# ch4r10t33r/zigz

Hardware: AMD Instinct MI355X
Metric: trace steps/sec proved (BabyBear, 2^20 RV64I trace) (higher is better)
Workload: dtype u32

## Files before the change

### zigz_amd/csrc/host_sponge_batch.cpp

```cpp
#include <immintrin.h>
#include <stdint.h>
#include <stdlib.h>
#include <string.h>

#include <algorithm>
#include <atomic>
#include <condition_variable>
#include <deque>
#include <mutex>
#include <thread>
#include <vector>

#include "field.hpp"
#include "host_hash.hpp"

namespace zk {

bool cpu_has_avx512f();

namespace {

constexpr int SLOTS = 8;
constexpr size_t RATE = 136;

const uint64_t RC8[24] = {
    0x0000000000000001ull, 0x0000000000008082ull, 0x800000000000808aull, 0x8000000080008000ull, 0x000000000000808bull,
    0x0000000080000001ull, 0x8000000080008081ull, 0x8000000000008009ull, 0x000000000000008aull, 0x0000000000000088ull,
    0x0000000080008009ull, 0x000000008000000aull, 0x000000008000808bull, 0x800000000000008bull, 0x8000000000008089ull,
    0x8000000000008003ull, 0x8000000000008002ull, 0x8000000000000080ull, 0x000000000000800aull, 0x800000008000000aull,
    0x8000000080008081ull, 0x8000000000008080ull, 0x0000000080000001ull, 0x8000000080008008ull};

__attribute__((target("avx512f"))) void keccak_f1600_x8(uint64_t st[25][SLOTS]) {
#define X8_X3(a, b, c) _mm512_ternarylogic_epi64((a), (b), (c), 0x96)
#define X8_CHI(a, b, c) _mm512_ternarylogic_epi64((a), (b), (c), 0xD2)
#define X8_ROL(a, n) _mm512_rol_epi64((a), (n))
#define X8_B(n, a, cm, rp) X8_ROL(X8_X3(a, cm, rp), n)
#define X8_LD(i) _mm512_load_si512(st[i])
    __m512i a0 = X8_LD(0), a1 = X8_LD(1), a2 = X8_LD(2), a3 = X8_LD(3), a4 = X8_LD(4), a5 = X8_LD(5), a6 = X8_LD(6), a7 = X8_LD(7);
    __m512i a8 = X8_LD(8), a9 = X8_LD(9), a10 = X8_LD(10), a11 = X8_LD(11), a12 = X8_LD(12), a13 = X8_LD(13), a14 = X8_LD(14);
    __m512i a15 = X8_LD(15), a16 = X8_LD(16), a17 = X8_LD(17), a18 = X8_LD(18), a19 = X8_LD(19), a20 = X8_LD(20), a21 = X8_LD(21);
    __m512i a22 = X8_LD(22), a23 = X8_LD(23), a24 = X8_LD(24);
#pragma unroll 2
    for (int r = 0; r < 24; r++) {
        const __m512i c0 = X8_X3(X8_X3(a0, a5, a10), a15, a20), c1 = X8_X3(X8_X3(a1, a6, a11), a16, a21);
        const __m512i c2 = X8_X3(X8_X3(a2, a7, a12), a17, a22), c3 = X8_X3(X8_X3(a3, a8, a13), a18, a23);
        const __m512i c4 = X8_X3(X8_X3(a4, a9, a14), a19, a24);
        const __m512i r0 = X8_ROL(c0, 1), r1 = X8_ROL(c1, 1), r2 = X8_ROL(c2, 1), r3 = X8_ROL(c3, 1), r4 = X8_ROL(c4, 1);
        const __m512i b00 = X8_X3(a0, c4, r1);
        const __m512i b10 = X8_B(1, a1, c0, r2), b20 = X8_B(62, a2, c1, r3), b05 = X8_B(28, a3, c2, r4), b15 = X8_B(27, a4, c3, r0);
        const __m512i b16 = X8_B(36, a5, c4, r1), b01 = X8_B(44, a6, c0, r2), b11 = X8_B(6, a7, c1, r3), b21 = X8_B(55, a8, c2, r4);
        const __m512i b06 = X8_B(20, a9, c3, r0), b07 = X8_B(3, a10, c4, r1), b17 = X8_B(10, a11, c0, r2), b02 = X8_B(43, a12, c1, r3);
        const __m512i b12 = X8_B(25, a13, c2, r4), b22 = X8_B(39, a14, c3, r0), b23 = X8_B(41, a15, c4, r1), b08 = X8_B(45, a16, c0, r2);
        const __m512i b18 = X8_B(15, a17, c1, r3), b03 = X8_B(21, a18, c2, r4), b13 = X8_B(8, a19, c3, r0), b14 = X8_B(18, a20, c4, r1);
        const __m512i b24 = X8_B(2, a21, c0, r2), b09 = X8_B(61, a22, c1, r3), b19 = X8_B(56, a23, c2, r4), b04 = X8_B(14, a24, c3, r0);
        a0 = _mm512_xor_si512(X8_CHI(b00, b01, b02), _mm512_set1_epi64((long long)RC8[r]));
        a1 = X8_CHI(b01, b02, b03); a2 = X8_CHI(b02, b03, b04); a3 = X8_CHI(b03, b04, b00); a4 = X8_CHI(b04, b00, b01);
        a5 = X8_CHI(b05, b06, b07); a6 = X8_CHI(b06, b07, b08); a7 = X8_CHI(b07, b08, b09); a8 = X8_CHI(b08, b09, b05);
        a9 = X8_CHI(b09, b05, b06); a10 = X8_CHI(b10, b11, b12); a11 = X8_CHI(b11, b12, b13); a12 = X8_CHI(b12, b13, b14);
        a13 = X8_CHI(b13, b14, b10); a14 = X8_CHI(b14, b10, b11); a15 = X8_CHI(b15, b16, b17); a16 = X8_CHI(b16, b17, b18);
        a17 = X8_CHI(b17, b18, b19); a18 = X8_CHI(b18, b19, b15); a19 = X8_CHI(b19, b15, b16); a20 = X8_CHI(b20, b21, b22);
        a21 = X8_CHI(b21, b22, b23); a22 = X8_CHI(b22, b23, b24); a23 = X8_CHI(b23, b24, b20); a24 = X8_CHI(b24, b20, b21);
    }
#define X8_ST(i, v) _mm512_store_si512(st[i], (v))
    X8_ST(0, a0); X8_ST(1, a1); X8_ST(2, a2); X8_ST(3, a3); X8_ST(4, a4); X8_ST(5, a5); X8_ST(6, a6); X8_ST(7, a7); X8_ST(8, a8);
    X8_ST(9, a9); X8_ST(10, a10); X8_ST(11, a11); X8_ST(12, a12); X8_ST(13, a13); X8_ST(14, a14); X8_ST(15, a15); X8_ST(16, a16);
    X8_ST(17, a17); X8_ST(18, a18); X8_ST(19, a19); X8_ST(20, a20); X8_ST(21, a21); X8_ST(22, a22); X8_ST(23, a23); X8_ST(24, a24);
}

struct Job {
    uint64_t *st;
    size_t *pos;
    const uint8_t *tag;
    size_t tag_len;
    uint64_t start, count;
    std::mutex m;
    std::condition_variable cv;
    bool done = false;
};

struct Stream {
    static constexpr size_t CHUNK_RECORDS = 272;
    Job *job = nullptr;
    uint64_t v = 0, left = 0;
    size_t rec = 0, rd = 0, wr = 0;
    uint8_t tmpl[32];
    std::vector<uint8_t> buf;

    void open(Job *j) {
        job = j;
        rec = j->tag_len + 8;
        v = j->start % (uint64_t)P;
        left = j->count;
        rd = wr = 0;
        memset(tmpl, 0, sizeof(tmpl));
        memcpy(tmpl, j->tag, j->tag_len < 24 ? j->tag_len : 24);
        buf.resize(CHUNK_RECORDS * rec + RATE + 64);
    }
    size_t avail() const { return wr - rd; }
    bool exhausted() const { return left == 0 && rd == wr; }
    void fill() {
        if (avail() >= RATE || left == 0) return;
        if (rd) {
            memmove(buf.data(), buf.data() + rd, wr - rd);
            wr -= rd;
            rd = 0;
        }
        size_t m = (buf.size() - wr - 32) / rec;
        if (m > left) m = (size_t)left;
        uint8_t *q = buf.data() + wr;
        const size_t tl = job->tag_len;
        if (tl <= 24) {
            for (size_t k = 0; k < m; k++, q += rec) {
                memcpy(q, tmpl, 32);
                memcpy(q + tl, &v, 8);
                if (++v == (uint64_t)P) v = 0;
            }
        } else {
            for (size_t k = 0; k < m; k++, q += rec) {
                memcpy(q, job->tag, tl);
                memcpy(q + tl, &v, 8);
                if (++v == (uint64_t)P) v = 0;
            }
        }
        wr += m * rec;
        left -= m;
    }
};

class Service {
  public:
    ~Service() { resize(0); }

    void resize(int n) {
        std::unique_lock<std::mutex> lk(m_);
        if (n < 0) n = 0;
        if (n > 0 && !cpu_has_avx512f()) n = 0;
        if ((int)threads_.size() == n) return;
        enabled_.store(false, std::memory_order_release);
        stop_ = true;
        cv_.notify_all();
        std::vector<std::thread> old;
        old.swap(threads_);
        lk.unlock();
        for (auto &t : old) t.join();
        lk.lock();
        stop_ = false;
        for (int i = 0; i < n; i++) threads_.emplace_back([this] { serve(); });
        enabled_.store(n > 0, std::memory_order_release);
    }
    bool enabled() const { return enabled_.load(std::memory_order_acquire); }

    bool run(Job &j) {
        {
            std::lock_guard<std::mutex> lk(m_);
            if (threads_.empty() || stop_) return false;
            queue_.push_back(&j);
            pending_.fetch_add(1, std::memory_order_release);
        }
        cv_.notify_one();
        std::unique_lock<std::mutex> lk(j.m);
        j.cv.wait(lk, [&] { return j.done; });
        return true;
    }

  private:
    void serve() {
        alignas(64) uint64_t S[25][SLOTS];
        memset(S, 0, sizeof(S));
        Stream slot[SLOTS];
        size_t pos[SLOTS] = {0};
        int active = 0;
        for (;;) {
            if (active == 0 || (active < SLOTS && pending_.load(std::memory_order_acquire) > 0)) {
                std::unique_lock<std::mutex> lk(m_);
                if (active == 0) cv_.wait(lk, [&] { return stop_ || !queue_.empty(); });
                if (stop_ && active == 0 && queue_.empty()) return;
                for (int s = 0; s < SLOTS && !queue_.empty(); s++) {
                    if (slot[s].job) continue;
                    Job *j = queue_.front();
                    queue_.pop_front();
                    pending_.fetch_sub(1, std::memory_order_relaxed);
                    slot[s].open(j);
                    pos[s] = *j->pos;
                    for (int w = 0; w < 25; w++) S[w][s] = j->st[w];
                    active++;
                }
            }
            if (active == 1 && pending_.load(std::memory_order_acquire) == 0) {
                int s = 0;
                while (!slot[s].job) s++;
                Stream &st = slot[s];
                if (pos[s] == 0) {
                    uint64_t one[25];
                    for (int w = 0; w < 25; w++) one[w] = S[w][s];
                    for (int k = 0; k < 64; k++) {
                        st.fill();
                        if (st.avail() < RATE) break;
                        const uint8_t *src = st.buf.data() + st.rd;
                        for (int w = 0; w < 17; w++) {
                            uint64_t x;
                            memcpy(&x, src + 8 * w, 8);
                            one[w] ^= x;
                        }
                        st.rd += RATE;
                        host_keccak_permute(one, 0);
                    }
                    for (int w = 0; w < 25; w++) S[w][s] = one[w];
                }
            }
            bool permute = false;
            for (int s = 0; s < SLOTS; s++) {
                Stream &st = slot[s];
                if (!st.job) continue;
                st.fill();
                const size_t need = RATE - pos[s];
                size_t n = st.avail() < need ? st.avail() : need;
                const uint8_t *src = st.buf.data() + st.rd;
                if (pos[s] == 0 && n == RATE) {
                    for (int w = 0; w < 17; w++) {
                        uint64_t x;
                        memcpy(&x, src + 8 * w, 8);
                        S[w][s] ^= x;
                    }
                } else if (n) {
                    uint8_t blk[RATE] = {0};
                    memcpy(blk + pos[s], src, n);
                    for (int w = 0; w < 17; w++) {
                        uint64_t x;
                        memcpy(&x, blk + 8 * w, 8);
                        S[w][s] ^= x;
                    }
                }
                st.rd += n;
                pos[s] += n;
                if (pos[s] == RATE) {
                    pos[s] = 0;
                    permute = true;
                } else {
                    retire(S, s, slot, pos);
                    active--;
                }
            }
            if (permute) keccak_f1600_x8(S);
            for (int s = 0; s < SLOTS; s++)
                if (slot[s].job && slot[s].exhausted() && pos[s] == 0) {
                    retire(S, s, slot, pos);
                    active--;
                }
        }
    }

    static void retire(uint64_t S[25][SLOTS], int s, Stream *slot, size_t *pos) {
        Job *j = slot[s].job;
        for (int w = 0; w < 25; w++) j->st[w] = S[w][s];
        *j->pos = pos[s];
        slot[s].job = nullptr;
        std::lock_guard<std::mutex> lk(j->m);
        j->done = true;
        j->cv.notify_one();
    }

    std::mutex m_;
    std::condition_variable cv_;
    std::deque<Job *> queue_;
    std::vector<std::thread> threads_;
    bool stop_ = false;
    std::atomic<int> pending_{0};
    std::atomic<bool> enabled_{false};
};

Service &service() {
    static Service s;
    return s;
}

}

void host_sponge_servers(int n) { service().resize(n); }
bool host_sponge_batching() { return service().enabled(); }

bool host_sponge_absorb_tagged(uint64_t st[25], size_t *pos, const uint8_t *tag, size_t tag_len, uint64_t start, uint64_t count) {
    Job j;
    j.st = st;
    j.pos = pos;
    j.tag = tag;
    j.tag_len = tag_len;
    j.start = start;
    j.count = count;
    return service().run(j);
}

void host_keccak_permute_x8(uint64_t st[25][8]) { keccak_f1600_x8(st); }

void flat_commit_batch(const uint32_t *const *ev, const size_t *n, size_t count, uint8_t (*out)[32]) {
    constexpr size_t WORDS = RATE / 8;
    auto one = [&](size_t i) {
        Sha3_256 h;
        for (size_t j = 0; j < n[i]; j++) h.update_le64(ev[i][j]);
        h.finalize(out[i]);
    };
    std::vector<std::thread> th;
    if (!cpu_has_avx512f()) {
        th.reserve(count);
        for (size_t i = 0; i < count; i++) th.emplace_back(one, i);
        for (auto &t : th) t.join();
        return;
    }
    std::vector<size_t> order(count);
    for (size_t i = 0; i < count; i++) order[i] = i;
    std::sort(order.begin(), order.end(), [&](size_t a, size_t b) { return n[a] > n[b]; });
    auto group = [&](size_t g0) {
        const size_t ns = count - g0 < (size_t)SLOTS ? count - g0 : (size_t)SLOTS;
        alignas(64) uint64_t st[25][SLOTS];
        memset(st, 0, sizeof(st));
        size_t full[SLOTS] = {0};
        size_t blocks = 0;
        for (size_t s = 0; s < ns; s++) {
            full[s] = n[order[g0 + s]] / WORDS;
            if (full[s] > blocks) blocks = full[s];
        }
        auto finish = [&](size_t s) {
            const size_t i = order[g0 + s];
            Sha3_256 h;
            for (int l = 0; l < 25; l++) h.raw_state()[l] = st[l][s];
            *h.raw_pos() = 0;
            for (size_t j = full[s] * WORDS; j < n[i]; j++) h.update_le64(ev[i][j]);
            h.finalize(out[i]);
        };
        for (size_t s = 0; s < ns; s++)
            if (full[s] == 0) finish(s);
        for (size_t b = 0; b < blocks; b++) {
            for (size_t s = 0; s < ns; s++) {
                if (b >= full[s]) continue;
                const uint32_t *v = ev[order[g0 + s]] + b * WORDS;
                for (size_t w = 0; w < WORDS; w++) st[w][s] ^= v[w];
            }
            keccak_f1600_x8(st);
            for (size_t s = 0; s < ns; s++)
                if (full[s] == b + 1) finish(s);
        }
    };
    const size_t groups = (count + SLOTS - 1) / SLOTS;
    th.reserve(groups);
    for (size_t g = 1; g < groups; g++) th.emplace_back(group, g * SLOTS);
    group(0);
    for (auto &t : th) t.join();
}

}
```

Measured before the change: 2.182 billion.

## Generate tagged sponge input in AVX-512 registers instead of staging byte buffers

The batched host Keccak sponge server no longer materialises tagged counter records into per-stream byte buffers. Streams with short tags now produce each 64-bit input lane directly in registers, using a gather from a per-slot tag table plus shifts of the running counter. Several absorb-and-permute blocks then run back-to-back with the state held in registers, up to a cap set by an environment variable. This removes the memmove/memcpy staging and the per-block state reloads, at the cost of more complex lane arithmetic and a gather per lane.

```diff
diff --git a/zigz_amd/csrc/host_sponge_batch.cpp b/zigz_amd/csrc/host_sponge_batch.cpp
--- a/zigz_amd/csrc/host_sponge_batch.cpp
+++ b/zigz_amd/csrc/host_sponge_batch.cpp
@@ -30,41 +30,97 @@
     0x8000000000008003ull, 0x8000000000008002ull, 0x8000000000000080ull, 0x000000000000800aull, 0x800000008000000aull,
     0x8000000080008081ull, 0x8000000000008080ull, 0x0000000080000001ull, 0x8000000080008008ull};
 
-__attribute__((target("avx512f"))) void keccak_f1600_x8(uint64_t st[25][SLOTS]) {
 #define X8_X3(a, b, c) _mm512_ternarylogic_epi64((a), (b), (c), 0x96)
 #define X8_CHI(a, b, c) _mm512_ternarylogic_epi64((a), (b), (c), 0xD2)
 #define X8_ROL(a, n) _mm512_rol_epi64((a), (n))
 #define X8_B(n, a, cm, rp) X8_ROL(X8_X3(a, cm, rp), n)
-#define X8_LD(i) _mm512_load_si512(st[i])
-    __m512i a0 = X8_LD(0), a1 = X8_LD(1), a2 = X8_LD(2), a3 = X8_LD(3), a4 = X8_LD(4), a5 = X8_LD(5), a6 = X8_LD(6), a7 = X8_LD(7);
-    __m512i a8 = X8_LD(8), a9 = X8_LD(9), a10 = X8_LD(10), a11 = X8_LD(11), a12 = X8_LD(12), a13 = X8_LD(13), a14 = X8_LD(14);
-    __m512i a15 = X8_LD(15), a16 = X8_LD(16), a17 = X8_LD(17), a18 = X8_LD(18), a19 = X8_LD(19), a20 = X8_LD(20), a21 = X8_LD(21);
-    __m512i a22 = X8_LD(22), a23 = X8_LD(23), a24 = X8_LD(24);
+#define X8_LOAD(st)                                                                                                          \
+    __m512i a0 = _mm512_load_si512(st[0]), a1 = _mm512_load_si512(st[1]), a2 = _mm512_load_si512(st[2]);                      \
+    __m512i a3 = _mm512_load_si512(st[3]), a4 = _mm512_load_si512(st[4]), a5 = _mm512_load_si512(st[5]);                      \
+    __m512i a6 = _mm512_load_si512(st[6]), a7 = _mm512_load_si512(st[7]), a8 = _mm512_load_si512(st[8]);                      \
+    __m512i a9 = _mm512_load_si512(st[9]), a10 = _mm512_load_si512(st[10]), a11 = _mm512_load_si512(st[11]);                  \
+    __m512i a12 = _mm512_load_si512(st[12]), a13 = _mm512_load_si512(st[13]), a14 = _mm512_load_si512(st[14]);                \
+    __m512i a15 = _mm512_load_si512(st[15]), a16 = _mm512_load_si512(st[16]), a17 = _mm512_load_si512(st[17]);                \
+    __m512i a18 = _mm512_load_si512(st[18]), a19 = _mm512_load_si512(st[19]), a20 = _mm512_load_si512(st[20]);                \
+    __m512i a21 = _mm512_load_si512(st[21]), a22 = _mm512_load_si512(st[22]), a23 = _mm512_load_si512(st[23]);                \
+    __m512i a24 = _mm512_load_si512(st[24])
+#define X8_ST(st, i, v) _mm512_store_si512(st[i], (v))
+#define X8_STORE(st)                                                                                                         \
+    X8_ST(st, 0, a0); X8_ST(st, 1, a1); X8_ST(st, 2, a2); X8_ST(st, 3, a3); X8_ST(st, 4, a4); X8_ST(st, 5, a5);               \
+    X8_ST(st, 6, a6); X8_ST(st, 7, a7); X8_ST(st, 8, a8); X8_ST(st, 9, a9); X8_ST(st, 10, a10); X8_ST(st, 11, a11);           \
+    X8_ST(st, 12, a12); X8_ST(st, 13, a13); X8_ST(st, 14, a14); X8_ST(st, 15, a15); X8_ST(st, 16, a16); X8_ST(st, 17, a17);   \
+    X8_ST(st, 18, a18); X8_ST(st, 19, a19); X8_ST(st, 20, a20); X8_ST(st, 21, a21); X8_ST(st, 22, a22); X8_ST(st, 23, a23);   \
+    X8_ST(st, 24, a24)
+#define X8_ROUND(rc)                                                                                                         \
+    {                                                                                                                        \
+        const __m512i c0 = X8_X3(X8_X3(a0, a5, a10), a15, a20), c1 = X8_X3(X8_X3(a1, a6, a11), a16, a21);                     \
+        const __m512i c2 = X8_X3(X8_X3(a2, a7, a12), a17, a22), c3 = X8_X3(X8_X3(a3, a8, a13), a18, a23);                     \
+        const __m512i c4 = X8_X3(X8_X3(a4, a9, a14), a19, a24);                                                              \
+        const __m512i r0 = X8_ROL(c0, 1), r1 = X8_ROL(c1, 1), r2 = X8_ROL(c2, 1), r3 = X8_ROL(c3, 1), r4 = X8_ROL(c4, 1);     \
+        const __m512i b00 = X8_X3(a0, c4, r1);                                                                               \
+        const __m512i b10 = X8_B(1, a1, c0, r2), b20 = X8_B(62, a2, c1, r3), b05 = X8_B(28, a3, c2, r4);                      \
+        const __m512i b15 = X8_B(27, a4, c3, r0), b16 = X8_B(36, a5, c4, r1), b01 = X8_B(44, a6, c0, r2);                     \
+        const __m512i b11 = X8_B(6, a7, c1, r3), b21 = X8_B(55, a8, c2, r4), b06 = X8_B(20, a9, c3, r0);                      \
+        const __m512i b07 = X8_B(3, a10, c4, r1), b17 = X8_B(10, a11, c0, r2), b02 = X8_B(43, a12, c1, r3);                   \
+        const __m512i b12 = X8_B(25, a13, c2, r4), b22 = X8_B(39, a14, c3, r0), b23 = X8_B(41, a15, c4, r1);                  \
+        const __m512i b08 = X8_B(45, a16, c0, r2), b18 = X8_B(15, a17, c1, r3), b03 = X8_B(21, a18, c2, r4);                  \
+        const __m512i b13 = X8_B(8, a19, c3, r0), b14 = X8_B(18, a20, c4, r1), b24 = X8_B(2, a21, c0, r2);                    \
+        const __m512i b09 = X8_B(61, a22, c1, r3), b19 = X8_B(56, a23, c2, r4), b04 = X8_B(14, a24, c3, r0);                  \
+        a0 = _mm512_xor_si512(X8_CHI(b00, b01, b02), _mm512_set1_epi64((long long)(rc)));                                    \
+        a1 = X8_CHI(b01, b02, b03); a2 = X8_CHI(b02, b03, b04); a3 = X8_CHI(b03, b04, b00); a4 = X8_CHI(b04, b00, b01);       \
+        a5 = X8_CHI(b05, b06, b07); a6 = X8_CHI(b06, b07, b08); a7 = X8_CHI(b07, b08, b09); a8 = X8_CHI(b08, b09, b05);       \
+        a9 = X8_CHI(b09, b05, b06); a10 = X8_CHI(b10, b11, b12); a11 = X8_CHI(b11, b12, b13); a12 = X8_CHI(b12, b13, b14);    \
+        a13 = X8_CHI(b13, b14, b10); a14 = X8_CHI(b14, b10, b11); a15 = X8_CHI(b15, b16, b17); a16 = X8_CHI(b16, b17, b18);   \
+        a17 = X8_CHI(b17, b18, b19); a18 = X8_CHI(b18, b19, b15); a19 = X8_CHI(b19, b15, b16); a20 = X8_CHI(b20, b21, b22);   \
+        a21 = X8_CHI(b21, b22, b23); a22 = X8_CHI(b22, b23, b24); a23 = X8_CHI(b23, b24, b20); a24 = X8_CHI(b24, b20, b21);   \
+    }
+
+__attribute__((target("avx512f"))) void keccak_f1600_x8(uint64_t st[25][SLOTS]) {
+    X8_LOAD(st);
 #pragma unroll 2
-    for (int r = 0; r < 24; r++) {
-        const __m512i c0 = X8_X3(X8_X3(a0, a5, a10), a15, a20), c1 = X8_X3(X8_X3(a1, a6, a11), a16, a21);
-        const __m512i c2 = X8_X3(X8_X3(a2, a7, a12), a17, a22), c3 = X8_X3(X8_X3(a3, a8, a13), a18, a23);
-        const __m512i c4 = X8_X3(X8_X3(a4, a9, a14), a19, a24);
-        const __m512i r0 = X8_ROL(c0, 1), r1 = X8_ROL(c1, 1), r2 = X8_ROL(c2, 1), r3 = X8_ROL(c3, 1), r4 = X8_ROL(c4, 1);
-        const __m512i b00 = X8_X3(a0, c4, r1);
-        const __m512i b10 = X8_B(1, a1, c0, r2), b20 = X8_B(62, a2, c1, r3), b05 = X8_B(28, a3, c2, r4), b15 = X8_B(27, a4, c3, r0);
-        const __m512i b16 = X8_B(36, a5, c4, r1), b01 = X8_B(44, a6, c0, r2), b11 = X8_B(6, a7, c1, r3), b21 = X8_B(55, a8, c2, r4);
-        const __m512i b06 = X8_B(20, a9, c3, r0), b07 = X8_B(3, a10, c4, r1), b17 = X8_B(10, a11, c0, r2), b02 = X8_B(43, a12, c1, r3);
-        const __m512i b12 = X8_B(25, a13, c2, r4), b22 = X8_B(39, a14, c3, r0), b23 = X8_B(41, a15, c4, r1), b08 = X8_B(45, a16, c0, r2);
-        const __m512i b18 = X8_B(15, a17, c1, r3), b03 = X8_B(21, a18, c2, r4), b13 = X8_B(8, a19, c3, r0), b14 = X8_B(18, a20, c4, r1);
-        const __m512i b24 = X8_B(2, a21, c0, r2), b09 = X8_B(61, a22, c1, r3), b19 = X8_B(56, a23, c2, r4), b04 = X8_B(14, a24, c3, r0);
-        a0 = _mm512_xor_si512(X8_CHI(b00, b01, b02), _mm512_set1_epi64((long long)RC8[r]));
-        a1 = X8_CHI(b01, b02, b03); a2 = X8_CHI(b02, b03, b04); a3 = X8_CHI(b03, b04, b00); a4 = X8_CHI(b04, b00, b01);
-        a5 = X8_CHI(b05, b06, b07); a6 = X8_CHI(b06, b07, b08); a7 = X8_CHI(b07, b08, b09); a8 = X8_CHI(b08, b09, b05);
-        a9 = X8_CHI(b09, b05, b06); a10 = X8_CHI(b10, b11, b12); a11 = X8_CHI(b11, b12, b13); a12 = X8_CHI(b12, b13, b14);
-        a13 = X8_CHI(b13, b14, b10); a14 = X8_CHI(b14, b10, b11); a15 = X8_CHI(b15, b16, b17); a16 = X8_CHI(b16, b17, b18);
-        a17 = X8_CHI(b17, b18, b19); a18 = X8_CHI(b18, b19, b15); a19 = X8_CHI(b19, b15, b16); a20 = X8_CHI(b20, b21, b22);
-        a21 = X8_CHI(b21, b22, b23); a22 = X8_CHI(b22, b23, b24); a23 = X8_CHI(b23, b24, b20); a24 = X8_CHI(b24, b20, b21);
-    }
-#define X8_ST(i, v) _mm512_store_si512(st[i], (v))
-    X8_ST(0, a0); X8_ST(1, a1); X8_ST(2, a2); X8_ST(3, a3); X8_ST(4, a4); X8_ST(5, a5); X8_ST(6, a6); X8_ST(7, a7); X8_ST(8, a8);
-    X8_ST(9, a9); X8_ST(10, a10); X8_ST(11, a11); X8_ST(12, a12); X8_ST(13, a13); X8_ST(14, a14); X8_ST(15, a15); X8_ST(16, a16);
-    X8_ST(17, a17); X8_ST(18, a18); X8_ST(19, a19); X8_ST(20, a20); X8_ST(21, a21); X8_ST(22, a22); X8_ST(23, a23); X8_ST(24, a24);
+    for (int r = 0; r < 24; r++) X8_ROUND(RC8[r]);
+    X8_STORE(st);
+}
+
+constexpr size_t LANE_TAG = 24;
+constexpr size_t TAB = LANE_TAG + 8;
+struct Lanes {
+    alignas(64) uint64_t v[SLOTS];
+    alignas(64) uint64_t r8[SLOTS];
+    alignas(64) uint64_t tl8[SLOTS], rec8[SLOTS];
+    alignas(64) uint64_t tab[SLOTS][TAB];
+};
+
+__attribute__((target("avx512f"))) void absorb_run(uint64_t S[25][SLOTS], Lanes &L, __mmask8 ready, size_t blocks) {
+    const __m512i tl8 = _mm512_load_si512(L.tl8), rec8 = _mm512_load_si512(L.rec8);
+    const __m512i base = _mm512_setr_epi64(0, 8 * TAB, 16 * TAB, 24 * TAB, 32 * TAB, 40 * TAB, 48 * TAB, 56 * TAB);
+    const __m512i p = _mm512_set1_epi64((long long)P), one = _mm512_set1_epi64(1), step = _mm512_set1_epi64(64);
+    __m512i v = _mm512_load_si512(L.v), r8 = _mm512_load_si512(L.r8);
+    X8_LOAD(S);
+#define X8_ABSORB(a)                                                                                                         \
+    {                                                                                                                        \
+        const __m512i t = _mm512_mask_i64gather_epi64(_mm512_setzero_si512(), ready, _mm512_add_epi64(base, r8), L.tab, 1);  \
+        const __m512i up = _mm512_sub_epi64(tl8, r8);                                                                        \
+        __m512i v1 = _mm512_add_epi64(v, one);                                                                               \
+        v1 = _mm512_maskz_mov_epi64(_mm512_cmpneq_epi64_mask(v1, p), v1);                                                    \
+        const __m512i c = _mm512_ternarylogic_epi64(_mm512_sllv_epi64(v, up), _mm512_srlv_epi64(v, _mm512_sub_epi64(r8, tl8)), \
+                                                    _mm512_sllv_epi64(v1, _mm512_add_epi64(up, rec8)), 0xFE);                \
+        a = _mm512_mask_ternarylogic_epi64(a, ready, t, c, 0x1E);                                           \
+        r8 = _mm512_add_epi64(r8, step);                                                                                     \
+        const __mmask8 next = _mm512_cmpge_epu64_mask(r8, rec8);                                                             \
+        r8 = _mm512_mask_sub_epi64(r8, next, r8, rec8);                                                                      \
+        v = _mm512_mask_mov_epi64(v, next, v1);                                                                              \
+    }
+    for (size_t b = 0; b < blocks; b++) {
+        X8_ABSORB(a0) X8_ABSORB(a1) X8_ABSORB(a2) X8_ABSORB(a3) X8_ABSORB(a4) X8_ABSORB(a5) X8_ABSORB(a6) X8_ABSORB(a7)
+        X8_ABSORB(a8) X8_ABSORB(a9) X8_ABSORB(a10) X8_ABSORB(a11) X8_ABSORB(a12) X8_ABSORB(a13) X8_ABSORB(a14)
+        X8_ABSORB(a15) X8_ABSORB(a16)
+#pragma unroll 2
+        for (int r = 0; r < 24; r++) X8_ROUND(RC8[r]);
+    }
+    X8_STORE(S);
+    _mm512_mask_store_epi64(L.v, ready, v);
+    _mm512_mask_store_epi64(L.r8, ready, r8);
 }
 
 struct Job {
@@ -78,52 +134,67 @@
     bool done = false;
 };
 
+constexpr size_t MAX_TAG = 248;
+
 struct Stream {
-    static constexpr size_t CHUNK_RECORDS = 272;
     Job *job = nullptr;
-    uint64_t v = 0, left = 0;
-    size_t rec = 0, rd = 0, wr = 0;
+    uint64_t *v = nullptr, *r8 = nullptr;
+    uint64_t rem = 0;
+    size_t rec = 0;
+    bool lanes = false;
     uint8_t tmpl[32];
-    std::vector<uint8_t> buf;
-
-    void open(Job *j) {
+
+    void open(Job *j, Lanes &L, int s) {
         job = j;
-        rec = j->tag_len + 8;
-        v = j->start % (uint64_t)P;
-        left = j->count;
-        rd = wr = 0;
+        const size_t tl = j->tag_len;
+        rec = tl + 8;
+        v = &L.v[s];
+        r8 = &L.r8[s];
+        *v = j->start % (uint64_t)P;
+        *r8 = 0;
+        rem = j->count * rec;
+        lanes = tl <= LANE_TAG;
         memset(tmpl, 0, sizeof(tmpl));
-        memcpy(tmpl, j->tag, j->tag_len < 24 ? j->tag_len : 24);
-        buf.resize(CHUNK_RECORDS * rec + RATE + 64);
-    }
-    size_t avail() const { return wr - rd; }
-    bool exhausted() const { return left == 0 && rd == wr; }
-    void fill() {
-        if (avail() >= RATE || left == 0) return;
-        if (rd) {
-            memmove(buf.data(), buf.data() + rd, wr - rd);
-            wr -= rd;
-            rd = 0;
-        }
-        size_t m = (buf.size() - wr - 32) / rec;
-        if (m > left) m = (size_t)left;
-        uint8_t *q = buf.data() + wr;
+        memcpy(tmpl, j->tag, lanes ? tl : LANE_TAG);
+        L.tl8[s] = 8 * tl;
+        L.rec8[s] = 8 * rec;
+        if (lanes) {
+            uint8_t img[2 * TAB + 8] = {0};
+            memcpy(img, j->tag, tl);
+            memcpy(img + rec, j->tag, tl);
+            for (size_t r = 0; r < rec; r++) memcpy(&L.tab[s][r], img + r, 8);
+        }
+    }
+    void take(uint8_t *dst, size_t n) {
         const size_t tl = job->tag_len;
-        if (tl <= 24) {
-            for (size_t k = 0; k < m; k++, q += rec) {
-                memcpy(q, tmpl, 32);
-                memcpy(q + tl, &v, 8);
-                if (++v == (uint64_t)P) v = 0;
-            }
-        } else {
-            for (size_t k = 0; k < m; k++, q += rec) {
-                memcpy(q, job->tag, tl);
-                memcpy(q + tl, &v, 8);
-                if (++v == (uint64_t)P) v = 0;
-            }
-        }
-        wr += m * rec;
-        left -= m;
+        size_t r = (size_t)(*r8 >> 3);
+        uint64_t c = *v;
+        rem -= n;
+        while (n) {
+            size_t m = rec;
+            if (r == 0 && lanes && n >= sizeof(tmpl)) {
+                memcpy(dst, tmpl, sizeof(tmpl));
+                memcpy(dst + tl, &c, 8);
+            } else if (r == 0 && n >= rec) {
+                memcpy(dst, job->tag, tl);
+                memcpy(dst + tl, &c, 8);
+            } else {
+                uint8_t one[MAX_TAG + 8];
+                memcpy(one, job->tag, tl);
+                memcpy(one + tl, &c, 8);
+                m = rec - r < n ? rec - r : n;
+                memcpy(dst, one + r, m);
+            }
+            dst += m;
+            n -= m;
+            r += m;
+            if (r == rec) {
+                r = 0;
+                if (++c == (uint64_t)P) c = 0;
+            }
+        }
+        *v = c;
+        *r8 = 8 * r;
     }
 };
 
@@ -167,9 +238,15 @@
     void serve() {
         alignas(64) uint64_t S[25][SLOTS];
         memset(S, 0, sizeof(S));
+        Lanes L;
+        memset(&L, 0, sizeof(L));
+        for (int s = 0; s < SLOTS; s++) L.rec8[s] = 64;
         Stream slot[SLOTS];
         size_t pos[SLOTS] = {0};
         int active = 0;
+        size_t run_cap = 32;
+        if (const char *e = getenv("ZIGZ_SPONGE_RUN_CAP"))
+            if (atoi(e) > 0) run_cap = (size_t)atoi(e);
         for (;;) {
             if (active == 0 || (active < SLOTS && pending_.load(std::memory_order_acquire) > 0)) {
                 std::unique_lock<std::mutex> lk(m_);
@@ -180,7 +257,7 @@
                     Job *j = queue_.front();
                     queue_.pop_front();
                     pending_.fetch_sub(1, std::memory_order_relaxed);
-                    slot[s].open(j);
+                    slot[s].open(j, L, s);
                     pos[s] = *j->pos;
                     for (int w = 0; w < 25; w++) S[w][s] = j->st[w];
                     active++;
@@ -190,48 +267,47 @@
                 int s = 0;
                 while (!slot[s].job) s++;
                 Stream &st = slot[s];
-                if (pos[s] == 0) {
+                if (pos[s] == 0 && st.rem >= RATE) {
                     uint64_t one[25];
                     for (int w = 0; w < 25; w++) one[w] = S[w][s];
-                    for (int k = 0; k < 64; k++) {
-                        st.fill();
-                        if (st.avail() < RATE) break;
-                        const uint8_t *src = st.buf.data() + st.rd;
+                    uint8_t chunk[64 * RATE];
+                    const size_t nb = st.rem / RATE < 64 ? (size_t)(st.rem / RATE) : 64;
+                    st.take(chunk, nb * RATE);
+                    for (size_t k = 0; k < nb; k++) {
+                        const uint8_t *src = chunk + k * RATE;
                         for (int w = 0; w < 17; w++) {
                             uint64_t x;
                             memcpy(&x, src + 8 * w, 8);
                             one[w] ^= x;
                         }
-                        st.rd += RATE;
                         host_keccak_permute(one, 0);
                     }
                     for (int w = 0; w < 25; w++) S[w][s] = one[w];
-                }
-            }
+                    if (st.rem >= RATE) continue;
+                }
+            }
+            __mmask8 ready = 0;
+            size_t blocks = run_cap;
             bool permute = false;
             for (int s = 0; s < SLOTS; s++) {
                 Stream &st = slot[s];
                 if (!st.job) continue;
-                st.fill();
+                if (st.lanes && pos[s] == 0 && st.rem >= RATE) {
+                    ready |= (__mmask8)(1u << s);
+                    if (st.rem / RATE < blocks) blocks = (size_t)(st.rem / RATE);
+                    continue;
+                }
                 const size_t need = RATE - pos[s];
-                size_t n = st.avail() < need ? st.avail() : need;
-                const uint8_t *src = st.buf.data() + st.rd;
-                if (pos[s] == 0 && n == RATE) {
-                    for (int w = 0; w < 17; w++) {
-                        uint64_t x;
-                        memcpy(&x, src + 8 * w, 8);
-                        S[w][s] ^= x;
-                    }
-                } else if (n) {
+                const size_t n = st.rem < need ? (size_t)st.rem : need;
+                if (n) {
                     uint8_t blk[RATE] = {0};
-                    memcpy(blk + pos[s], src, n);
+                    st.take(blk + pos[s], n);
                     for (int w = 0; w < 17; w++) {
                         uint64_t x;
                         memcpy(&x, blk + 8 * w, 8);
                         S[w][s] ^= x;
                     }
                 }
-                st.rd += n;
                 pos[s] += n;
                 if (pos[s] == RATE) {
                     pos[s] = 0;
@@ -241,9 +317,16 @@
                     active--;
                 }
             }
-            if (permute) keccak_f1600_x8(S);
+            if (ready) {
+                if (permute) blocks = 1;
+                absorb_run(S, L, ready, blocks);
+                for (int s = 0; s < SLOTS; s++)
+                    if (ready >> s & 1) slot[s].rem -= blocks * RATE;
+            } else if (permute) {
+                keccak_f1600_x8(S);
+            }
             for (int s = 0; s < SLOTS; s++)
-                if (slot[s].job && slot[s].exhausted() && pos[s] == 0) {
+                if (slot[s].job && slot[s].rem == 0 && pos[s] == 0) {
                     retire(S, s, slot, pos);
                     active--;
                 }
@@ -280,6 +363,7 @@
 bool host_sponge_batching() { return service().enabled(); }
 
 bool host_sponge_absorb_tagged(uint64_t st[25], size_t *pos, const uint8_t *tag, size_t tag_len, uint64_t start, uint64_t count) {
+    if (tag_len > MAX_TAG) return false;
     Job j;
     j.st = st;
     j.pos = pos;
```

Result: faster. 2.309 billion, median of 6 (+5.8%).

## Generate sponge blocks directly from precomputed shapes and batch multi-block Keccak runs

Applied to the files above, without the earlier changes.

Drops the buffered record stream and its memmove/memcpy refill. Each rate block is now synthesized directly with AVX-512 shifts from per-offset precomputed templates (BlockShape). A new run_blocks loop keeps all 8 sponge states in registers across up to 32 absorbs, transposing the generated rows into the lane layout, and polls the pending queue so it can exit early. The Keccak round is restructured as a ping-pong two-round helper. This adds a lot of complex bit-shifting logic that must match the old byte stream exactly, including wraparound near P.

```diff
diff --git a/zigz_amd/csrc/host_sponge_batch.cpp b/zigz_amd/csrc/host_sponge_batch.cpp
--- a/zigz_amd/csrc/host_sponge_batch.cpp
+++ b/zigz_amd/csrc/host_sponge_batch.cpp
@@ -30,41 +30,50 @@
     0x8000000000008003ull, 0x8000000000008002ull, 0x8000000000000080ull, 0x000000000000800aull, 0x800000008000000aull,
     0x8000000080008081ull, 0x8000000000008080ull, 0x0000000080000001ull, 0x8000000080008008ull};
 
-__attribute__((target("avx512f"))) void keccak_f1600_x8(uint64_t st[25][SLOTS]) {
+#define X8_TARGET __attribute__((target("avx512f")))
+#define X8_INLINE X8_TARGET __attribute__((always_inline)) inline
 #define X8_X3(a, b, c) _mm512_ternarylogic_epi64((a), (b), (c), 0x96)
 #define X8_CHI(a, b, c) _mm512_ternarylogic_epi64((a), (b), (c), 0xD2)
 #define X8_ROL(a, n) _mm512_rol_epi64((a), (n))
-#define X8_B(n, a, cm, rp) X8_ROL(X8_X3(a, cm, rp), n)
-#define X8_LD(i) _mm512_load_si512(st[i])
-    __m512i a0 = X8_LD(0), a1 = X8_LD(1), a2 = X8_LD(2), a3 = X8_LD(3), a4 = X8_LD(4), a5 = X8_LD(5), a6 = X8_LD(6), a7 = X8_LD(7);
-    __m512i a8 = X8_LD(8), a9 = X8_LD(9), a10 = X8_LD(10), a11 = X8_LD(11), a12 = X8_LD(12), a13 = X8_LD(13), a14 = X8_LD(14);
-    __m512i a15 = X8_LD(15), a16 = X8_LD(16), a17 = X8_LD(17), a18 = X8_LD(18), a19 = X8_LD(19), a20 = X8_LD(20), a21 = X8_LD(21);
-    __m512i a22 = X8_LD(22), a23 = X8_LD(23), a24 = X8_LD(24);
-#pragma unroll 2
-    for (int r = 0; r < 24; r++) {
-        const __m512i c0 = X8_X3(X8_X3(a0, a5, a10), a15, a20), c1 = X8_X3(X8_X3(a1, a6, a11), a16, a21);
-        const __m512i c2 = X8_X3(X8_X3(a2, a7, a12), a17, a22), c3 = X8_X3(X8_X3(a3, a8, a13), a18, a23);
-        const __m512i c4 = X8_X3(X8_X3(a4, a9, a14), a19, a24);
-        const __m512i r0 = X8_ROL(c0, 1), r1 = X8_ROL(c1, 1), r2 = X8_ROL(c2, 1), r3 = X8_ROL(c3, 1), r4 = X8_ROL(c4, 1);
-        const __m512i b00 = X8_X3(a0, c4, r1);
-        const __m512i b10 = X8_B(1, a1, c0, r2), b20 = X8_B(62, a2, c1, r3), b05 = X8_B(28, a3, c2, r4), b15 = X8_B(27, a4, c3, r0);
-        const __m512i b16 = X8_B(36, a5, c4, r1), b01 = X8_B(44, a6, c0, r2), b11 = X8_B(6, a7, c1, r3), b21 = X8_B(55, a8, c2, r4);
-        const __m512i b06 = X8_B(20, a9, c3, r0), b07 = X8_B(3, a10, c4, r1), b17 = X8_B(10, a11, c0, r2), b02 = X8_B(43, a12, c1, r3);
-        const __m512i b12 = X8_B(25, a13, c2, r4), b22 = X8_B(39, a14, c3, r0), b23 = X8_B(41, a15, c4, r1), b08 = X8_B(45, a16, c0, r2);
-        const __m512i b18 = X8_B(15, a17, c1, r3), b03 = X8_B(21, a18, c2, r4), b13 = X8_B(8, a19, c3, r0), b14 = X8_B(18, a20, c4, r1);
-        const __m512i b24 = X8_B(2, a21, c0, r2), b09 = X8_B(61, a22, c1, r3), b19 = X8_B(56, a23, c2, r4), b04 = X8_B(14, a24, c3, r0);
-        a0 = _mm512_xor_si512(X8_CHI(b00, b01, b02), _mm512_set1_epi64((long long)RC8[r]));
-        a1 = X8_CHI(b01, b02, b03); a2 = X8_CHI(b02, b03, b04); a3 = X8_CHI(b03, b04, b00); a4 = X8_CHI(b04, b00, b01);
-        a5 = X8_CHI(b05, b06, b07); a6 = X8_CHI(b06, b07, b08); a7 = X8_CHI(b07, b08, b09); a8 = X8_CHI(b08, b09, b05);
-        a9 = X8_CHI(b09, b05, b06); a10 = X8_CHI(b10, b11, b12); a11 = X8_CHI(b11, b12, b13); a12 = X8_CHI(b12, b13, b14);
-        a13 = X8_CHI(b13, b14, b10); a14 = X8_CHI(b14, b10, b11); a15 = X8_CHI(b15, b16, b17); a16 = X8_CHI(b16, b17, b18);
-        a17 = X8_CHI(b17, b18, b19); a18 = X8_CHI(b18, b19, b15); a19 = X8_CHI(b19, b15, b16); a20 = X8_CHI(b20, b21, b22);
-        a21 = X8_CHI(b21, b22, b23); a22 = X8_CHI(b22, b23, b24); a23 = X8_CHI(b23, b24, b20); a24 = X8_CHI(b24, b20, b21);
-    }
-#define X8_ST(i, v) _mm512_store_si512(st[i], (v))
-    X8_ST(0, a0); X8_ST(1, a1); X8_ST(2, a2); X8_ST(3, a3); X8_ST(4, a4); X8_ST(5, a5); X8_ST(6, a6); X8_ST(7, a7); X8_ST(8, a8);
-    X8_ST(9, a9); X8_ST(10, a10); X8_ST(11, a11); X8_ST(12, a12); X8_ST(13, a13); X8_ST(14, a14); X8_ST(15, a15); X8_ST(16, a16);
-    X8_ST(17, a17); X8_ST(18, a18); X8_ST(19, a19); X8_ST(20, a20); X8_ST(21, a21); X8_ST(22, a22); X8_ST(23, a23); X8_ST(24, a24);
+#define X8_XOR(a, b) _mm512_xor_si512((a), (b))
+
+X8_INLINE void keccak_round_x8(const __m512i (&a)[25], __m512i (&e)[25], uint64_t rc) {
+    const __m512i c0 = X8_X3(X8_X3(a[0], a[5], a[10]), a[15], a[20]), c1 = X8_X3(X8_X3(a[1], a[6], a[11]), a[16], a[21]);
+    const __m512i c2 = X8_X3(X8_X3(a[2], a[7], a[12]), a[17], a[22]), c3 = X8_X3(X8_X3(a[3], a[8], a[13]), a[18], a[23]);
+    const __m512i c4 = X8_X3(X8_X3(a[4], a[9], a[14]), a[19], a[24]);
+    const __m512i d0 = X8_XOR(c4, X8_ROL(c1, 1)), d1 = X8_XOR(c0, X8_ROL(c2, 1)), d2 = X8_XOR(c1, X8_ROL(c3, 1));
+    const __m512i d3 = X8_XOR(c2, X8_ROL(c4, 1)), d4 = X8_XOR(c3, X8_ROL(c0, 1));
+    __m512i b0, b1, b2, b3, b4;
+#define X8_BD(i, x, n) X8_ROL(X8_XOR(a[i], d##x), n)
+#define X8_CHI5(y)                                                                                                      \
+    e[y] = X8_CHI(b0, b1, b2); e[y + 1] = X8_CHI(b1, b2, b3); e[y + 2] = X8_CHI(b2, b3, b4); e[y + 3] = X8_CHI(b3, b4, b0); \
+    e[y + 4] = X8_CHI(b4, b0, b1)
+    b0 = X8_XOR(a[0], d0); b1 = X8_BD(6, 1, 44); b2 = X8_BD(12, 2, 43); b3 = X8_BD(18, 3, 21); b4 = X8_BD(24, 4, 14);
+    X8_CHI5(0);
+    e[0] = X8_XOR(e[0], _mm512_set1_epi64((long long)rc));
+    b0 = X8_BD(3, 3, 28); b1 = X8_BD(9, 4, 20); b2 = X8_BD(10, 0, 3); b3 = X8_BD(16, 1, 45); b4 = X8_BD(22, 2, 61);
+    X8_CHI5(5);
+    b0 = X8_BD(1, 1, 1); b1 = X8_BD(7, 2, 6); b2 = X8_BD(13, 3, 25); b3 = X8_BD(19, 4, 8); b4 = X8_BD(20, 0, 18);
+    X8_CHI5(10);
+    b0 = X8_BD(4, 4, 27); b1 = X8_BD(5, 0, 36); b2 = X8_BD(11, 1, 10); b3 = X8_BD(17, 2, 15); b4 = X8_BD(23, 3, 56);
+    X8_CHI5(15);
+    b0 = X8_BD(2, 2, 62); b1 = X8_BD(8, 3, 55); b2 = X8_BD(14, 4, 39); b3 = X8_BD(15, 0, 41); b4 = X8_BD(21, 1, 2);
+    X8_CHI5(20);
+}
+
+X8_INLINE void keccak_rounds_x8(__m512i (&a)[25]) {
+    __m512i e[25];
+    for (int r = 0; r < 24; r += 2) {
+        keccak_round_x8(a, e, RC8[r]);
+        keccak_round_x8(e, a, RC8[r + 1]);
+    }
+}
+
+X8_TARGET void keccak_f1600_x8(uint64_t st[25][SLOTS]) {
+    __m512i a[25];
+    for (int i = 0; i < 25; i++) a[i] = _mm512_load_si512(st[i]);
+    keccak_rounds_x8(a);
+    for (int i = 0; i < 25; i++) _mm512_store_si512(st[i], a[i]);
 }
 
 struct Job {
@@ -78,54 +87,153 @@
     bool done = false;
 };
 
+struct BlockShape {
+    alignas(64) uint64_t tmpl[17];
+    uint8_t adv, next;
+    alignas(8) uint8_t d[24], sl[24], sr[24], sn[24];
+};
+constexpr size_t FAST_REC = 64;
+
 struct Stream {
-    static constexpr size_t CHUNK_RECORDS = 272;
     Job *job = nullptr;
-    uint64_t v = 0, left = 0;
-    size_t rec = 0, rd = 0, wr = 0;
-    uint8_t tmpl[32];
-    std::vector<uint8_t> buf;
+    const uint8_t *tag = nullptr;
+    size_t tl = 0, rec = 0, r = 0;
+    uint64_t v = 0, rem = 0;
+    uint64_t span = 0;
+    bool shaped = false;
+    std::vector<BlockShape> shape;
 
     void open(Job *j) {
         job = j;
-        rec = j->tag_len + 8;
+        tag = j->tag;
+        tl = j->tag_len;
+        rec = tl + 8;
+        r = 0;
         v = j->start % (uint64_t)P;
-        left = j->count;
-        rd = wr = 0;
-        memset(tmpl, 0, sizeof(tmpl));
-        memcpy(tmpl, j->tag, j->tag_len < 24 ? j->tag_len : 24);
-        buf.resize(CHUNK_RECORDS * rec + RATE + 64);
-    }
-    size_t avail() const { return wr - rd; }
-    bool exhausted() const { return left == 0 && rd == wr; }
-    void fill() {
-        if (avail() >= RATE || left == 0) return;
-        if (rd) {
-            memmove(buf.data(), buf.data() + rd, wr - rd);
-            wr -= rd;
-            rd = 0;
-        }
-        size_t m = (buf.size() - wr - 32) / rec;
-        if (m > left) m = (size_t)left;
-        uint8_t *q = buf.data() + wr;
-        const size_t tl = job->tag_len;
-        if (tl <= 24) {
-            for (size_t k = 0; k < m; k++, q += rec) {
-                memcpy(q, tmpl, 32);
-                memcpy(q + tl, &v, 8);
+        rem = j->count * rec;
+        span = RATE / rec + 2;
+        shaped = rec <= FAST_REC;
+        if (!shaped) return;
+        shape.resize(rec);
+        for (size_t r0 = 0; r0 < rec; r0++) {
+            BlockShape &b = shape[r0];
+            memset(&b, 0, sizeof(b));
+            b.adv = (uint8_t)((r0 + RATE) / rec);
+            b.next = (uint8_t)((r0 + RATE) % rec);
+            for (size_t w = 0; w < 24; w++) b.sl[w] = b.sn[w] = 64;
+            for (size_t w = 0; w < 17; w++) {
+                const size_t q = (r0 + 8 * w) % rec;
+                uint8_t t[8];
+                for (size_t i = 0; i < 8; i++) t[i] = (q + i) % rec < tl ? tag[(q + i) % rec] : 0;
+                memcpy(&b.tmpl[w], t, 8);
+                b.d[w] = (uint8_t)((r0 + 8 * w) / rec);
+                if (q > tl) b.sl[w] = 0, b.sr[w] = (uint8_t)(8 * (q - tl));
+                else if (tl - q < 8) b.sl[w] = (uint8_t)(8 * (tl - q));
+                if (rec - q + tl < 8) b.sn[w] = (uint8_t)(8 * (rec - q + tl));
+            }
+        }
+    }
+    bool exhausted() const { return rem == 0; }
+
+    void read(uint8_t *dst, size_t n) {
+        rem -= n;
+        while (n) {
+            size_t c;
+            if (r < tl) {
+                c = tl - r < n ? tl - r : n;
+                memcpy(dst, tag + r, c);
+            } else {
+                c = rec - r < n ? rec - r : n;
+                memcpy(dst, (const uint8_t *)&v + (r - tl), c);
+            }
+            dst += c;
+            n -= c;
+            r += c;
+            if (r == rec) {
+                r = 0;
                 if (++v == (uint64_t)P) v = 0;
             }
-        } else {
-            for (size_t k = 0; k < m; k++, q += rec) {
-                memcpy(q, job->tag, tl);
-                memcpy(q + tl, &v, 8);
-                if (++v == (uint64_t)P) v = 0;
-            }
-        }
-        wr += m * rec;
-        left -= m;
+        }
+    }
+    uint64_t shaped_blocks() const { return shaped ? std::min(rem / RATE, ((uint64_t)P - 1 - v) / span) : 0; }
+    static uint64_t shl(uint64_t x, unsigned n) { return n < 64 ? x << n : 0; }
+    uint64_t word(const BlockShape &b, size_t w) const {
+        const uint64_t c = v + b.d[w];
+        return b.tmpl[w] ^ (shl(c, b.sl[w]) >> b.sr[w]) ^ shl(c + 1, b.sn[w]);
+    }
+    void advance(const BlockShape &b) {
+        v += b.adv;
+        r = b.next;
+        rem -= RATE;
+    }
+    X8_INLINE void block_x8(uint64_t out[17]) {
+        const BlockShape &b = shape[r];
+        const __m512i vv = _mm512_set1_epi64((long long)v), one = _mm512_set1_epi64(1);
+        for (int h = 0; h < 16; h += 8) {
+#define X8_LD8(p) _mm512_cvtepu8_epi64(_mm_loadl_epi64((const __m128i *)(p)))
+            const __m512i c = _mm512_add_epi64(vv, X8_LD8(b.d + h));
+            const __m512i x = _mm512_srlv_epi64(_mm512_sllv_epi64(c, X8_LD8(b.sl + h)), X8_LD8(b.sr + h));
+            const __m512i y = _mm512_sllv_epi64(_mm512_add_epi64(c, one), X8_LD8(b.sn + h));
+            _mm512_storeu_si512(out + h, X8_X3(_mm512_load_si512(b.tmpl + h), x, y));
+        }
+        out[16] = word(b, 16);
+        advance(b);
     }
 };
+
+X8_INLINE void transpose_x8(const uint64_t (*rows)[24], int c0, __m512i (&t)[8]) {
+    __m512i p[8], q[8];
+    for (int i = 0; i < 8; i += 2) {
+        const __m512i lo = _mm512_load_si512(rows[i] + c0), hi = _mm512_load_si512(rows[i + 1] + c0);
+        p[i] = _mm512_unpacklo_epi64(lo, hi);
+        p[i + 1] = _mm512_unpackhi_epi64(lo, hi);
+    }
+    for (int k = 0; k < 2; k++) {
+        q[k] = _mm512_shuffle_i64x2(p[k], p[2 + k], 0x88);
+        q[2 + k] = _mm512_shuffle_i64x2(p[k], p[2 + k], 0xdd);
+        q[4 + k] = _mm512_shuffle_i64x2(p[4 + k], p[6 + k], 0x88);
+        q[6 + k] = _mm512_shuffle_i64x2(p[4 + k], p[6 + k], 0xdd);
+        t[k] = _mm512_shuffle_i64x2(q[k], q[4 + k], 0x88);
+        t[4 + k] = _mm512_shuffle_i64x2(q[k], q[4 + k], 0xdd);
+        t[2 + k] = _mm512_shuffle_i64x2(q[2 + k], q[6 + k], 0x88);
+        t[6 + k] = _mm512_shuffle_i64x2(q[2 + k], q[6 + k], 0xdd);
+    }
+}
+
+X8_TARGET __attribute__((noinline)) void run_blocks(uint64_t S[25][SLOTS], Stream *slot, int n, const std::atomic<int> *poll) {
+    alignas(64) uint64_t rows[SLOTS][24];
+    alignas(64) uint64_t last[SLOTS];
+    memset(rows, 0, sizeof(rows));
+    memset(last, 0, sizeof(last));
+    __m512i a[25];
+    for (int i = 0; i < 25; i++) a[i] = _mm512_load_si512(S[i]);
+    for (int k = 0; k < n; k++) {
+        for (int s = 0; s < SLOTS; s++)
+            if (slot[s].job) {
+                slot[s].block_x8(rows[s]);
+                last[s] = rows[s][16];
+            }
+        __m512i t[8];
+        transpose_x8(rows, 0, t);
+        for (int i = 0; i < 8; i++) a[i] = X8_XOR(a[i], t[i]);
+        transpose_x8(rows, 8, t);
+        for (int i = 0; i < 8; i++) a[8 + i] = X8_XOR(a[8 + i], t[i]);
+        a[16] = X8_XOR(a[16], _mm512_load_si512(last));
+        keccak_rounds_x8(a);
+        if (poll && poll->load(std::memory_order_relaxed) > 0) break;
+    }
+    for (int i = 0; i < 25; i++) _mm512_store_si512(S[i], a[i]);
+}
+
+X8_TARGET void lone_blocks(Stream &st, uint64_t one[25], int n) {
+    for (; n > 0 && st.rem >= RATE; n--) {
+        alignas(64) uint64_t blk[17];
+        if (st.shaped_blocks()) st.block_x8(blk);
+        else st.read((uint8_t *)blk, RATE);
+        for (int w = 0; w < 17; w++) one[w] ^= blk[w];
+        host_keccak_permute(one, 0);
+    }
+}
 
 class Service {
   public:
@@ -164,6 +272,8 @@
     }
 
   private:
+    static constexpr int RUN_STEPS = 32;
+
     void serve() {
         alignas(64) uint64_t S[25][SLOTS];
         memset(S, 0, sizeof(S));
@@ -193,45 +303,33 @@
                 if (pos[s] == 0) {
                     uint64_t one[25];
                     for (int w = 0; w < 25; w++) one[w] = S[w][s];
-                    for (int k = 0; k < 64; k++) {
-                        st.fill();
-                        if (st.avail() < RATE) break;
-                        const uint8_t *src = st.buf.data() + st.rd;
-                        for (int w = 0; w < 17; w++) {
-                            uint64_t x;
-                            memcpy(&x, src + 8 * w, 8);
-                            one[w] ^= x;
-                        }
-                        st.rd += RATE;
-                        host_keccak_permute(one, 0);
-                    }
+                    lone_blocks(st, one, 64);
                     for (int w = 0; w < 25; w++) S[w][s] = one[w];
+                    if (st.rem >= RATE) continue;
                 }
+            }
+            uint64_t run = active ? RUN_STEPS : 0;
+            for (int s = 0; s < SLOTS; s++)
+                if (slot[s].job) run = std::min(run, pos[s] == 0 ? slot[s].shaped_blocks() : 0);
+            if (run) {
+                run_blocks(S, slot, (int)run, active < SLOTS ? &pending_ : nullptr);
+                continue;
             }
             bool permute = false;
             for (int s = 0; s < SLOTS; s++) {
                 Stream &st = slot[s];
                 if (!st.job) continue;
-                st.fill();
                 const size_t need = RATE - pos[s];
-                size_t n = st.avail() < need ? st.avail() : need;
-                const uint8_t *src = st.buf.data() + st.rd;
-                if (pos[s] == 0 && n == RATE) {
-                    for (int w = 0; w < 17; w++) {
-                        uint64_t x;
-                        memcpy(&x, src + 8 * w, 8);
-                        S[w][s] ^= x;
-                    }
-                } else if (n) {
-                    uint8_t blk[RATE] = {0};
-                    memcpy(blk + pos[s], src, n);
+                const size_t n = st.rem < need ? (size_t)st.rem : need;
+                if (n) {
+                    alignas(8) uint8_t blk[RATE] = {0};
+                    st.read(blk + pos[s], n);
                     for (int w = 0; w < 17; w++) {
                         uint64_t x;
                         memcpy(&x, blk + 8 * w, 8);
                         S[w][s] ^= x;
                     }
                 }
-                st.rd += n;
                 pos[s] += n;
                 if (pos[s] == RATE) {
                     pos[s] = 0;
```

New measurement: 2.306 billion before, 2.320 billion after (median of 6 runs). Within noise of the previous version (+0.6%).
